# Youngju-Na/UFORecon

Measured on AMD Instinct MI355X. Metric: rays/s (per-ray volume-rendering path, 64+64 hierarchical samples, DTU-shaped 3-view 512x640), higher is better.
Workload: dtype f32; 1 GPU; configs[1]: full 512x640 frame = 327680 rays, 3 source views, 64+64 samples, rays sharded by row tiles over 1 GPU(s), depth/RGB tiles all-gathered; rays_per_frame=327680, chunk_rays=4096, side_streams=3

## Files before the change

### uforecon_amd/csrc/gather.hip

```cpp
#include <algorithm>
#include <cstdlib>
#include "ufr_device.h"
#include "ufr_internal.h"
#include "volume_sample.h"

namespace ufr {

__device__ __forceinline__ f32x4 lerp_tap4_buf(__amdgpu_buffer_rsrc_t r, unsigned base, int stride_bytes, const Tap2& t, unsigned c4) {
  f32x4 v[4];
#pragma unroll
  for (int k = 0; k < 4; ++k)
    v[k] = buf_ld4(r, t.o[k] >= 0 ? base + __umul24((unsigned)t.o[k], (unsigned)stride_bytes) + c4 : kBufOut);
  f32x4 acc;
#pragma unroll
  for (int e = 0; e < 4; ++e) {
    float a = mul_rn(v[0][e], t.w[0]);
    a = fmaf(v[1][e], t.w[1], a);
    a = fmaf(v[2][e], t.w[2], a);
    acc[e] = fmaf(v[3][e], t.w[3], a);
  }
  return acc;
}

typedef int i32x4 __attribute__((ext_vector_type(4)));

__device__ __forceinline__ void put_tap(float* dst, const Tap2& t) {
  *reinterpret_cast<i32x4*>(dst) = i32x4{t.o[0], t.o[1], t.o[2], t.o[3]};
  *reinterpret_cast<f32x4*>(dst + 4) = f32x4{t.w[0], t.w[1], t.w[2], t.w[3]};
}
__device__ __forceinline__ Tap2 get_tap(const float* src) {
  const i32x4 o = *reinterpret_cast<const i32x4*>(src);
  const f32x4 w = *reinterpret_cast<const f32x4*>(src + 4);
  Tap2 t;
#pragma unroll
  for (int k = 0; k < 4; ++k) { t.o[k] = o[k]; t.w[k] = w[k]; }
  return t;
}

__device__ __forceinline__ void presim_block(const PreSim& ps, const float* sim, int sim_stride, float* out, int out_stride,
                                             int lane) {
  const int g = lane >> 4, j = lane & 15;
  f32x4 h1[4][2], h2[4][2], o[4];
  float x0[4][2];
#pragma unroll
  for (int u = 0; u < 4; ++u) {
    const float* sq = sim + (16 * u + j) * sim_stride;
    x0[u][0] = sq[g];
    x0[u][1] = sq[4 + g];
  }
  {
    float a1[2][2];
#pragma unroll
    for (int to = 0; to < 2; ++to) {
#pragma unroll
      for (int s = 0; s < 2; ++s) a1[to][s] = ps.w0[(16 * to + j) * 8 + 4 * s + g];
      const f32x4 b1 = ld4(ps.b0 + 16 * to + 4 * g);
#pragma unroll
      for (int u = 0; u < 4; ++u) h1[u][to] = b1;
    }
#pragma unroll
    for (int s = 0; s < 2; ++s)
#pragma unroll
      for (int to = 0; to < 2; ++to)
#pragma unroll
        for (int u = 0; u < 4; ++u) h1[u][to] = mfma16(a1[to][s], x0[u][s], h1[u][to]);
  }
  {
    float a2[2][2][4];
#pragma unroll
    for (int to = 0; to < 2; ++to) {
#pragma unroll
      for (int ti = 0; ti < 2; ++ti)
#pragma unroll
        for (int r = 0; r < 4; ++r) a2[to][ti][r] = ps.w2[(16 * to + j) * 32 + 16 * ti + 4 * g + r];
      const f32x4 b2 = ld4(ps.b2 + 16 * to + 4 * g);
#pragma unroll
      for (int u = 0; u < 4; ++u) h2[u][to] = b2;
    }
#pragma unroll
    for (int ti = 0; ti < 2; ++ti)
#pragma unroll
      for (int r = 0; r < 4; ++r)
#pragma unroll
        for (int to = 0; to < 2; ++to)
#pragma unroll
          for (int u = 0; u < 4; ++u) h2[u][to] = mfma16(a2[to][ti][r], fmaxf(h1[u][ti][r], 0.f), h2[u][to]);
  }
  {
    float a3[2][4];
#pragma unroll
    for (int to = 0; to < 2; ++to)
#pragma unroll
      for (int r = 0; r < 4; ++r) a3[to][r] = ps.w4[j * 32 + 16 * to + 4 * g + r];
    const f32x4 b3 = ld4(ps.b4 + 4 * g);
#pragma unroll
    for (int u = 0; u < 4; ++u) o[u] = b3;
#pragma unroll
    for (int ti = 0; ti < 2; ++ti)
#pragma unroll
      for (int r = 0; r < 4; ++r)
#pragma unroll
        for (int u = 0; u < 4; ++u) o[u] = mfma16(a3[ti][r], fmaxf(h2[u][ti][r], 0.f), o[u]);
  }
#pragma unroll
  for (int u = 0; u < 4; ++u) st4(out + (16 * u + j) * out_stride + 24 + 4 * g, o[u]);
}

constexpr int kGatherMinW = 5;

#ifdef UFR_PHASE_TIMING
__device__ unsigned long long g_gather_phase[32];
#define UFR_G_PHASE(i)                                                                 \
  {                                                                                    \
    const unsigned long long t_now = __builtin_readcyclecounter();                     \
    g_acc[i] = t_now - g_prev;                                                         \
    g_prev = t_now;                                                                    \
  }
#else
#define UFR_G_PHASE(i)
#endif

template <int NVT>
__global__ void __launch_bounds__(64 * NVT, kGatherMinW) gather_kernel(FrameDev f, PreSim ps, const float* __restrict__ ray_o,
                                                      int o_stride, const float* __restrict__ ray_d,
                                                      const float* __restrict__ zval, int P, int SN,
                                                      float* __restrict__ x_tokens, float* __restrict__ x_point,
                                                      float* __restrict__ rgb_out,
                                                      float* __restrict__ dir_out, float* __restrict__ sim8_out,
                                                      float* __restrict__ vol24_out, float* __restrict__ xy_out,
                                                      float* __restrict__ maskz_out,
                                                      const float* __restrict__ vol24_in,
                                                      const float* __restrict__ sim8_in) {
  extern __shared__ __attribute__((aligned(16))) float smem[];
  constexpr int NV = NVT;
  constexpr int npair = NV * (NV - 1) / 2;
  float* sh_sim = smem;
  float* sh_tapF = sh_sim + 64 * npair * 8;
  float* sh_tapM = sh_tapF + NV * 64 * 8;
  float* sh_vol = sh_tapF;
  constexpr int sim_slot = npair * 8;
  constexpr bool out_in_sim = sim_slot >= 48;
  float* sh_out = out_in_sim ? sh_sim + 8 : sh_tapF;
  constexpr int out_stride = out_in_sim ? sim_slot : 40;
#ifdef UFR_PHASE_TIMING
  unsigned long long g_acc[8] = {};
  unsigned long long g_prev = __builtin_readcyclecounter();
#endif

  const int v = threadIdx.x >> 6, p = threadIdx.x & 63;
  const int vu = __builtin_amdgcn_readfirstlane(v);
  const int nb8 = (int)(gridDim.x / 8) * 8;
  const int blk = (int)blockIdx.x < nb8 ? (int)(blockIdx.x % 8) * (nb8 / 8) + (int)(blockIdx.x / 8) : (int)blockIdx.x;
  const int pidx = blk * 64 + p;
  const bool active = pidx < P;
  const int pc = active ? pidx : P - 1;
  const int ray = pc / SN;

  const float zz = zval[pc];
  const float* o = ray_o + (size_t)ray * o_stride;
  const float px = mul_add_unfused(zz, ray_d[3 * ray + 0], o[0]);
  const float py = mul_add_unfused(zz, ray_d[3 * ray + 1], o[1]);
  const float pz = mul_add_unfused(zz, ray_d[3 * ray + 2], o[2]);

  const float* M = f.pose[v];
  float qx = fmaf(M[2], pz, fmaf(M[1], py, mul_rn(M[0], px))) + M[3];
  float qy = fmaf(M[6], pz, fmaf(M[5], py, mul_rn(M[4], px))) + M[7];
  float qz = fmaf(M[10], pz, fmaf(M[9], py, mul_rn(M[8], px))) + M[11];
  const float mask_z = qz > 0.f ? 1.f : 0.f;
  const float x = qx / qz, y = qy / qz;
  if (active && xy_out) {
    xy_out[((size_t)v * P + pidx) * 2 + 0] = x;
    xy_out[((size_t)v * P + pidx) * 2 + 1] = y;
  }
  if (active && maskz_out) maskz_out[(size_t)v * P + pidx] = mask_z;

  const int row_cols = x_point ? kViewCols : UFR_TOKEN_DIM, pe_col = x_point ? 32 : 72;
  float* xrow = x_tokens + ((size_t)pc * NV + v) * row_cols;

  {
    put_tap(sh_tapF + (v * 64 + p) * 8, taps_zeros(unnorm2d_nac(x, f.w), unnorm2d_nac(y, f.h), f.w, f.h));
    put_tap(sh_tapM + (v * 64 + p) * 8, taps_border(unnorm2d_ac(x, f.w), unnorm2d_ac(y, f.h), f.w, f.h));
    Tap2 tf = taps_zeros(unnorm2d_nac(x, f.W), unnorm2d_nac(y, f.H), f.W, f.H);
    const unsigned img_px = (unsigned)(f.H * f.W);
    f32x4 c4 = lerp_tap4_buf(buf_rsrc(f.rgb + (size_t)vu * img_px * 4, img_px * 16u), 0u, 16, tf, 0u);
    const float inb = (x <= 1.f && x >= -1.f && y <= 1.f && y >= -1.f) ? 1.f : 0.f;
    c4[3] = inb * mask_z;
    if (active) st4(rgb_out + ((size_t)pidx * NV + v) * 4, c4);
    float dv[4];
    const __amdgpu_buffer_rsrc_t rdepth = buf_rsrc(f.depth + (size_t)vu * img_px, img_px * 4u);
#pragma unroll
    for (int k = 0; k < 4; ++k) dv[k] = buf_ld1(rdepth, tf.o[k] >= 0 ? (unsigned)tf.o[k] * 4u : kBufOut);
    const float dm = fmaf(dv[3], tf.w[3], fmaf(dv[2], tf.w[2], fmaf(dv[1], tf.w[1], mul_rn(dv[0], tf.w[0]))));
    const float* R = f.w2c_z[v];
    float zc = fmaf(R[2], pz, fmaf(R[1], py, mul_rn(R[0], px))) + R[3];
    float delta = dm - zc;
    float pe[8];
#pragma unroll
    for (int k = 0; k < 4; ++k) {
      const float fr = 3.14159274101257324f * (float)(1 << k);
      pe[2 * k] = sinf(mul_rn(delta, fr));
      pe[2 * k + 1] = sinf(fmaf(delta, fr, 1.57079637050628662f));
    }
    if (active) {
      st4(xrow + pe_col, f32x4{pe[0], pe[1], pe[2], pe[3]});
      st4(xrow + pe_col + 4, f32x4{pe[4], pe[5], pe[6], pe[7]});
    }
    float ax = px - f.ref_pos[0], ay = py - f.ref_pos[1], az = pz - f.ref_pos[2];
    float bx = px - f.cam_pos[v][0], by = py - f.cam_pos[v][1], bz = pz - f.cam_pos[v][2];
    const float ra = __builtin_amdgcn_rcpf(sqrtf(ax * ax + ay * ay + az * az));
    const float rb = __builtin_amdgcn_rcpf(sqrtf(bx * bx + by * by + bz * bz));
    if (active) st4(dir_out + ((size_t)pidx * NV + v) * 4, f32x4{ax * ra - bx * rb, ay * ra - by * rb, az * ra - bz * rb, 0.f});
  }

  __syncthreads();
  UFR_G_PHASE(0)

  const int c8 = threadIdx.x & 7, grp = threadIdx.x >> 3;
  constexpr int n_grp = 64 * NV / 8;
  const unsigned map_px = (unsigned)(f.h * f.w);
  const __amdgpu_buffer_rsrc_t rfeat = buf_rsrc(f.feat, (unsigned)NV * map_px * 128u);
  const __amdgpu_buffer_rsrc_t rmatch = buf_rsrc(f.match, (unsigned)NV * map_px * (unsigned)f.match_ch * 4u);
  for (int item = grp; item < 64 * NV; item += n_grp) {
    const int ip = item / NV, iv = item - ip * NV;
    const int ipidx = blk * 64 + ip;
    if (ipidx < P) {
      const Tap2 t = get_tap(sh_tapF + (iv * 64 + ip) * 8);
      st4(x_tokens + ((size_t)ipidx * NV + iv) * row_cols + 4 * c8,
          lerp_tap4_buf(rfeat, (unsigned)iv * map_px * 128u, 128, t, 16u * c8));
    }
  }
  if (!sim8_in)
  for (int item = grp; item < 64 * npair; item += n_grp) {
    const int ip = item / npair, q = item - ip * npair;
    int a = 0, rem = q;
    while (rem >= NV - 1 - a) { rem -= NV - 1 - a; ++a; }
    const int b = a + rem;
    const int va = a, ca = b, vb = b + 1, cb = a;
    const Tap2 ta = get_tap(sh_tapM + (va * 64 + ip) * 8), tb = get_tap(sh_tapM + (vb * 64 + ip) * 8);
    const unsigned mrow = (unsigned)f.match_ch * 4u;
    f32x4 fa = lerp_tap4_buf(rmatch, (unsigned)va * map_px * mrow + 128u * ca, (int)mrow, ta, 16u * c8);
    f32x4 fb = lerp_tap4_buf(rmatch, (unsigned)vb * map_px * mrow + 128u * cb, (int)mrow, tb, 16u * c8);
    float na = fmaxf(sqrtf(fa[0] * fa[0] + fa[1] * fa[1] + fa[2] * fa[2] + fa[3] * fa[3]), 1e-8f);
    float nb = fmaxf(sqrtf(fb[0] * fb[0] + fb[1] * fb[1] + fb[2] * fb[2] + fb[3] * fb[3]), 1e-8f);
    const float ra = __builtin_amdgcn_rcpf(na), rb = __builtin_amdgcn_rcpf(nb);
    sh_sim[(ip * npair + q) * 8 + c8] = (fa[0] * ra) * (fb[0] * rb) + (fa[1] * ra) * (fb[1] * rb) +
                                        (fa[2] * ra) * (fb[2] * rb) + (fa[3] * ra) * (fb[3] * rb);
  }
  __syncthreads();
  UFR_G_PHASE(1)

  float own[25];
  if (vol24_in) {
#pragma unroll
    for (int c = 0; c < 25; ++c) own[c] = 0.f;
  } else {
    const float zn = ((qz - f.vol_near) / (f.vol_far - f.vol_near)) * 2.f - 1.f;
    float fl[24], wl = 0.f;
#pragma unroll
    for (int s = 0; s < UFR_NUM_STAGES; ++s) {
      float fs[8], ws;
      const float* vol = f.vol[s];
      const unsigned vox = (unsigned)(f.vD[s] * f.vH[s] * f.vW[s]);
      sample_volume_buf(buf_rsrc(vol + (size_t)vu * vox * kVolCh, vox * (unsigned)(kVolCh * 4)), f.vD[s], f.vH[s], f.vW[s], x, y, zn,
                        fs, ws);
#pragma unroll
      for (int c = 0; c < 8; ++c) fl[8 * s + c] = fs[c];
      wl = s == 0 ? ws : wl + ws;
    }
#pragma unroll
    for (int c = 0; c < 24; ++c) own[c] = fl[c] * wl;
    own[24] = wl;
    if (v > 0) {
      float* dst = sh_vol + (p * (NV - 1) + (v - 1)) * 25;
#pragma unroll
      for (int c = 0; c < 25; ++c) dst[c] = own[c];
    }
  }
  __syncthreads();
  UFR_G_PHASE(2)

  if (v == 0) {
    float sim[8];
#pragma unroll
    for (int gi = 0; gi < 8; ++gi) {
      float s = 0.f;
      for (int q = 0; q < npair; ++q) s += sh_sim[(p * npair + q) * 8 + gi];
      sim[gi] = s / (float)npair;
      if (sim8_in) sim[gi] = sim8_in[(size_t)pc * 8 + gi];
    }
    {
      float Wsum = own[24];
      for (int n = 1; n < NV; ++n) Wsum += sh_vol[(p * (NV - 1) + n - 1) * 25 + 24];
      const float rW = 1.f / (Wsum + 1e-8f);
#pragma unroll
      for (int c = 0; c < 24; ++c) {
        float G = own[c];
        for (int n = 1; n < NV; ++n) G += sh_vol[(p * (NV - 1) + n - 1) * 25 + c];
        own[c] = G * rW;
        if (vol24_in) own[c] = vol24_in[(size_t)pc * 24 + c];
      }
    }
    __builtin_amdgcn_fence(__ATOMIC_RELEASE, "wavefront");
    __builtin_amdgcn_wave_barrier();
    __builtin_amdgcn_fence(__ATOMIC_ACQUIRE, "wavefront");
    float* mine = sh_sim + p * sim_slot;
    st4(mine, f32x4{sim[0], sim[1], sim[2], sim[3]});
    st4(mine + 4, f32x4{sim[4], sim[5], sim[6], sim[7]});
    float* ov = sh_out + p * out_stride;
#pragma unroll
    for (int c = 0; c < 24; c += 4) st4(ov + c, f32x4{own[c], own[c + 1], own[c + 2], own[c + 3]});
    UFR_G_PHASE(3)
    __builtin_amdgcn_fence(__ATOMIC_RELEASE, "wavefront");
    __builtin_amdgcn_wave_barrier();
    __builtin_amdgcn_fence(__ATOMIC_ACQUIRE, "wavefront");
    presim_block(ps, sh_sim, sim_slot, sh_out, out_stride, p);
  }
  __syncthreads();
  UFR_G_PHASE(4)

  const int npts = P - blk * 64 < 64 ? P - blk * 64 : 64;
  if (x_point) {
    float* dst = x_point + (size_t)blk * 64 * kPointCols;
    for (int i = threadIdx.x; i < npts * 10; i += 64 * NV) {
      const int ip = i / 10, c = i - ip * 10;
      st4(dst + 4 * i, ld4(sh_out + ip * out_stride + 4 * c));
    }
  } else {
    for (int i = threadIdx.x; i < npts * NV * 10; i += 64 * NV) {
      const int row = i / 10, c = i - row * 10;
      st4(x_tokens + ((size_t)blk * 64 * NV + row) * UFR_TOKEN_DIM + 32 + 4 * c, ld4(sh_out + (row / NV) * out_stride + 4 * c));
    }
  }
  if (vol24_out)
    for (int i = threadIdx.x; i < npts * 24; i += 64 * NV) {
      const int ip = i / 24;
      vol24_out[(size_t)blk * 64 * 24 + i] = sh_out[ip * out_stride + (i - ip * 24)];
    }
  if (sim8_out)
    for (int i = threadIdx.x; i < npts * 8; i += 64 * NV) sim8_out[(size_t)blk * 64 * 8 + i] = sh_sim[(i >> 3) * sim_slot + (i & 7)];
  UFR_G_PHASE(5)
#ifdef UFR_PHASE_TIMING
  if (threadIdx.x == 0) {
    for (int i = 0; i < 6; ++i) atomicAdd(&g_gather_phase[i], g_acc[i]);
    atomicAdd(&g_gather_phase[6], 1ull);
  }
#endif
}

hipError_t launch_gather(const FrameDev& f, const PreSim& ps, const float* ray_o, int o_stride, const float* ray_d,
                         const float* z, int RN, int SN, float* x_tokens, float* x_point, float* rgb, float* dir, float* sim8,
                         float* vol24, float* xy, float* mask_z, const float* vol24_in, const float* sim8_in,
                         hipStream_t s) {
  const int P = RN * SN, NV = f.NV;
  const int npair = NV * (NV - 1) / 2;
  const size_t taps = 2 * (size_t)NV * 64 * 8, volp = (size_t)64 * (NV - 1) * 25, outv = npair * 8 >= 48 ? 0 : 64 * 40;
  size_t lds = sizeof(float) * ((size_t)64 * npair * 8 + std::max(std::max(taps, volp), outv));
  switch (NV) {
#define UFR_GATHER_CASE(N)                                                                                                   \
    case N:                                                                                                                  \
      hipLaunchKernelGGL(gather_kernel<N>, dim3((P + 63) / 64), dim3(64 * N), lds, s, f, ps, ray_o, o_stride, ray_d, z, P, SN, \
                         x_tokens, x_point, rgb, dir, sim8, vol24, xy, mask_z, vol24_in, sim8_in);                          \
      break;
    UFR_GATHER_CASE(2) UFR_GATHER_CASE(3) UFR_GATHER_CASE(4) UFR_GATHER_CASE(5) UFR_GATHER_CASE(6) UFR_GATHER_CASE(7)
#undef UFR_GATHER_CASE
    default: return hipErrorInvalidValue;
  }
  return hipGetLastError();
}

}

#ifdef UFR_PHASE_TIMING
extern "C" int ufr_debug_gather_phases(unsigned long long* out, int n, int reset) {
  unsigned long long h[32] = {};
  if (hipMemcpyFromSymbol(h, HIP_SYMBOL(ufr::g_gather_phase), sizeof(h)) != hipSuccess) return -1;
  for (int i = 0; i < n && i < 32; ++i) out[i] = h[i];
  if (reset) {
    unsigned long long z[32] = {};
    if (hipMemcpyToSymbol(HIP_SYMBOL(ufr::g_gather_phase), z, sizeof(z)) != hipSuccess) return -1;
  }
  return 0;
}
#endif
```

Before: 2.661 million rays/s.

## Cut gather kernel register pressure to raise occupancy for few-view configs

Splits the presim MLP block into two rolled halves of two 16-point groups so fewer accumulator registers are live at once. Per-view volume samples are now written straight to LDS, including view 0, instead of being held in a 25-float register array, and the reduction reads every partial from shared memory. Launch bounds request 8 waves per SIMD when there are 3 or fewer views. The goal is higher occupancy, paid for with more LDS traffic, a larger volume scratch area, and less MFMA overlap inside presim.

```diff
diff --git a/uforecon_amd/csrc/gather.hip b/uforecon_amd/csrc/gather.hip
--- a/uforecon_amd/csrc/gather.hip
+++ b/uforecon_amd/csrc/gather.hip
@@ -40,73 +40,78 @@
 __device__ __forceinline__ void presim_block(const PreSim& ps, const float* sim, int sim_stride, float* out, int out_stride,
                                              int lane) {
   const int g = lane >> 4, j = lane & 15;
-  f32x4 h1[4][2], h2[4][2], o[4];
-  float x0[4][2];
-#pragma unroll
-  for (int u = 0; u < 4; ++u) {
-    const float* sq = sim + (16 * u + j) * sim_stride;
-    x0[u][0] = sq[g];
-    x0[u][1] = sq[4 + g];
-  }
-  {
-    float a1[2][2];
-#pragma unroll
-    for (int to = 0; to < 2; ++to) {
-#pragma unroll
-      for (int s = 0; s < 2; ++s) a1[to][s] = ps.w0[(16 * to + j) * 8 + 4 * s + g];
-      const f32x4 b1 = ld4(ps.b0 + 16 * to + 4 * g);
-#pragma unroll
-      for (int u = 0; u < 4; ++u) h1[u][to] = b1;
-    }
-#pragma unroll
-    for (int s = 0; s < 2; ++s)
+#pragma unroll 1
+  for (int u0 = 0; u0 < 4; u0 += 2) {
+    asm volatile("" ::: "memory");
+    f32x4 h1[2][2], h2[2][2], o[2];
+    float x0[2][2];
+#pragma unroll
+    for (int u = 0; u < 2; ++u) {
+      const float* sq = sim + (16 * (u0 + u) + j) * sim_stride;
+      x0[u][0] = sq[g];
+      x0[u][1] = sq[4 + g];
+    }
+    {
+      float a1[2][2];
+#pragma unroll
+      for (int to = 0; to < 2; ++to) {
+#pragma unroll
+        for (int s = 0; s < 2; ++s) a1[to][s] = ps.w0[(16 * to + j) * 8 + 4 * s + g];
+        const f32x4 b1 = ld4(ps.b0 + 16 * to + 4 * g);
+#pragma unroll
+        for (int u = 0; u < 2; ++u) h1[u][to] = b1;
+      }
+#pragma unroll
+      for (int s = 0; s < 2; ++s)
+#pragma unroll
+        for (int to = 0; to < 2; ++to)
+#pragma unroll
+          for (int u = 0; u < 2; ++u) h1[u][to] = mfma16(a1[to][s], x0[u][s], h1[u][to]);
+    }
+    {
+      float a2[2][2][4];
+#pragma unroll
+      for (int to = 0; to < 2; ++to) {
+#pragma unroll
+        for (int ti = 0; ti < 2; ++ti)
+#pragma unroll
+          for (int r = 0; r < 4; ++r) a2[to][ti][r] = ps.w2[(16 * to + j) * 32 + 16 * ti + 4 * g + r];
+        const f32x4 b2 = ld4(ps.b2 + 16 * to + 4 * g);
+#pragma unroll
+        for (int u = 0; u < 2; ++u) h2[u][to] = b2;
+      }
+#pragma unroll
+      for (int ti = 0; ti < 2; ++ti)
+#pragma unroll
+        for (int r = 0; r < 4; ++r)
+#pragma unroll
+          for (int to = 0; to < 2; ++to)
+#pragma unroll
+            for (int u = 0; u < 2; ++u) h2[u][to] = mfma16(a2[to][ti][r], fmaxf(h1[u][ti][r], 0.f), h2[u][to]);
+    }
+    {
+      float a3[2][4];
 #pragma unroll
       for (int to = 0; to < 2; ++to)
 #pragma unroll
-        for (int u = 0; u < 4; ++u) h1[u][to] = mfma16(a1[to][s], x0[u][s], h1[u][to]);
-  }
-  {
-    float a2[2][2][4];
-#pragma unroll
-    for (int to = 0; to < 2; ++to) {
+        for (int r = 0; r < 4; ++r) a3[to][r] = ps.w4[j * 32 + 16 * to + 4 * g + r];
+      const f32x4 b3 = ld4(ps.b4 + 4 * g);
+#pragma unroll
+      for (int u = 0; u < 2; ++u) o[u] = b3;
 #pragma unroll
       for (int ti = 0; ti < 2; ++ti)
 #pragma unroll
-        for (int r = 0; r < 4; ++r) a2[to][ti][r] = ps.w2[(16 * to + j) * 32 + 16 * ti + 4 * g + r];
-      const f32x4 b2 = ld4(ps.b2 + 16 * to + 4 * g);
-#pragma unroll
-      for (int u = 0; u < 4; ++u) h2[u][to] = b2;
-    }
-#pragma unroll
-    for (int ti = 0; ti < 2; ++ti)
-#pragma unroll
-      for (int r = 0; r < 4; ++r)
-#pragma unroll
-        for (int to = 0; to < 2; ++to)
-#pragma unroll
-          for (int u = 0; u < 4; ++u) h2[u][to] = mfma16(a2[to][ti][r], fmaxf(h1[u][ti][r], 0.f), h2[u][to]);
-  }
-  {
-    float a3[2][4];
-#pragma unroll
-    for (int to = 0; to < 2; ++to)
-#pragma unroll
-      for (int r = 0; r < 4; ++r) a3[to][r] = ps.w4[j * 32 + 16 * to + 4 * g + r];
-    const f32x4 b3 = ld4(ps.b4 + 4 * g);
-#pragma unroll
-    for (int u = 0; u < 4; ++u) o[u] = b3;
-#pragma unroll
-    for (int ti = 0; ti < 2; ++ti)
-#pragma unroll
-      for (int r = 0; r < 4; ++r)
-#pragma unroll
-        for (int u = 0; u < 4; ++u) o[u] = mfma16(a3[ti][r], fmaxf(h2[u][ti][r], 0.f), o[u]);
-  }
-#pragma unroll
-  for (int u = 0; u < 4; ++u) st4(out + (16 * u + j) * out_stride + 24 + 4 * g, o[u]);
+        for (int r = 0; r < 4; ++r)
+#pragma unroll
+          for (int u = 0; u < 2; ++u) o[u] = mfma16(a3[ti][r], fmaxf(h2[u][ti][r], 0.f), o[u]);
+    }
+#pragma unroll
+    for (int u = 0; u < 2; ++u) st4(out + (16 * (u0 + u) + j) * out_stride + 24 + 4 * g, o[u]);
+  }
 }
 
 constexpr int kGatherMinW = 5;
+constexpr int kGatherMinWFew = 8;
 
 #ifdef UFR_PHASE_TIMING
 __device__ unsigned long long g_gather_phase[32];
@@ -121,7 +126,7 @@
 #endif
 
 template <int NVT>
-__global__ void __launch_bounds__(64 * NVT, kGatherMinW) gather_kernel(FrameDev f, PreSim ps, const float* __restrict__ ray_o,
+__global__ void __launch_bounds__(64 * NVT, NVT <= 3 ? kGatherMinWFew : kGatherMinW) gather_kernel(FrameDev f, PreSim ps, const float* __restrict__ ray_o,
                                                       int o_stride, const float* __restrict__ ray_d,
                                                       const float* __restrict__ zval, int P, int SN,
                                                       float* __restrict__ x_tokens, float* __restrict__ x_point,
@@ -249,13 +254,10 @@
   __syncthreads();
   UFR_G_PHASE(1)
 
-  float own[25];
-  if (vol24_in) {
-#pragma unroll
-    for (int c = 0; c < 25; ++c) own[c] = 0.f;
-  } else {
+  if (!vol24_in) {
     const float zn = ((qz - f.vol_near) / (f.vol_far - f.vol_near)) * 2.f - 1.f;
-    float fl[24], wl = 0.f;
+    float* dst = sh_vol + (p * NV + v) * 25;
+    float wl = 0.f;
 #pragma unroll
     for (int s = 0; s < UFR_NUM_STAGES; ++s) {
       float fs[8], ws;
@@ -264,17 +266,12 @@
       sample_volume_buf(buf_rsrc(vol + (size_t)vu * vox * kVolCh, vox * (unsigned)(kVolCh * 4)), f.vD[s], f.vH[s], f.vW[s], x, y, zn,
                         fs, ws);
 #pragma unroll
-      for (int c = 0; c < 8; ++c) fl[8 * s + c] = fs[c];
+      for (int c = 0; c < 8; ++c) dst[8 * s + c] = fs[c];
       wl = s == 0 ? ws : wl + ws;
     }
 #pragma unroll
-    for (int c = 0; c < 24; ++c) own[c] = fl[c] * wl;
-    own[24] = wl;
-    if (v > 0) {
-      float* dst = sh_vol + (p * (NV - 1) + (v - 1)) * 25;
-#pragma unroll
-      for (int c = 0; c < 25; ++c) dst[c] = own[c];
-    }
+    for (int c = 0; c < 24; ++c) dst[c] = dst[c] * wl;
+    dst[24] = wl;
   }
   __syncthreads();
   UFR_G_PHASE(2)
@@ -288,16 +285,20 @@
       sim[gi] = s / (float)npair;
       if (sim8_in) sim[gi] = sim8_in[(size_t)pc * 8 + gi];
     }
-    {
-      float Wsum = own[24];
-      for (int n = 1; n < NV; ++n) Wsum += sh_vol[(p * (NV - 1) + n - 1) * 25 + 24];
+    float own[24];
+    if (vol24_in) {
+#pragma unroll
+      for (int c = 0; c < 24; ++c) own[c] = vol24_in[(size_t)pc * 24 + c];
+    } else {
+      const float* part = sh_vol + p * NV * 25;
+      float Wsum = part[24];
+      for (int n = 1; n < NV; ++n) Wsum += part[n * 25 + 24];
       const float rW = 1.f / (Wsum + 1e-8f);
 #pragma unroll
       for (int c = 0; c < 24; ++c) {
-        float G = own[c];
-        for (int n = 1; n < NV; ++n) G += sh_vol[(p * (NV - 1) + n - 1) * 25 + c];
+        float G = part[c];
+        for (int n = 1; n < NV; ++n) G += part[n * 25 + c];
         own[c] = G * rW;
-        if (vol24_in) own[c] = vol24_in[(size_t)pc * 24 + c];
       }
     }
     __builtin_amdgcn_fence(__ATOMIC_RELEASE, "wavefront");
@@ -353,7 +354,7 @@
                          hipStream_t s) {
   const int P = RN * SN, NV = f.NV;
   const int npair = NV * (NV - 1) / 2;
-  const size_t taps = 2 * (size_t)NV * 64 * 8, volp = (size_t)64 * (NV - 1) * 25, outv = npair * 8 >= 48 ? 0 : 64 * 40;
+  const size_t taps = 2 * (size_t)NV * 64 * 8, volp = (size_t)64 * NV * 25, outv = npair * 8 >= 48 ? 0 : 64 * 40;
   size_t lds = sizeof(float) * ((size_t)64 * npair * 8 + std::max(std::max(taps, volp), outv));
   switch (NV) {
 #define UFR_GATHER_CASE(N)                                                                                                   \
```

Measured after the change: 2.659 million rays/s. No clear change (-0.1%).
